# KrArunT/whisper-rust-ort

Hardware: AMD Instinct MI355X
Metric: rtfx: audio seconds transcribed per wall second (whisper-base, 30 s clips, greedy 128 new tokens) (higher is better)
Workload: dtype bf16

## Files before the change

### whisper-rust-ort_amd/csrc/wh_cross_es.hip

```cpp
#include <stdlib.h>

#include <algorithm>

#include "wh_common.h"
#include "wh_es_common.h"
#include "wh_kernels.h"

namespace {

using namespace wh_es;

constexpr int ES_D = D, ES_H = H;
constexpr int ES_ROWB = ES_D * 2;
constexpr Format ES_F = {32, 32 * ES_ROWB, 4, true, 36};

template <int AUX, int NL, int ABL = 0, bool BEAM = false>
__global__ __launch_bounds__(256 + 64 * NL, 1) void k_dec_cross_attn_es(const float* __restrict__ qe, const bf16* __restrict__ E,
                                                                         bf16* __restrict__ out, int S, int e_rows, int mpad, int B, unsigned long long* dbg,
                                                                         int rows_per_clip) {
    constexpr int TK = ES_F.tk, TILEB = ES_F.tileb, SCP = ES_F.scp;
    static_assert(NL == 1 || NL == 2, "one or two loader waves");
    extern __shared__ __attribute__((aligned(16))) char smem[];
    float* sc = carve<ES_F>(smem).sc;
    float* Qs = carve<ES_F>(smem).Qs;
// ... 187 lines not shown
#pragma unroll
        for (int u = 0; u < 8; u++) {
            const float v = u < 4 ? a[u & 3] : b[u & 3];
            const bf16 hi = (bf16)v;
            xh[ks][u] = hi;
            xl[ks][u] = (bf16)(v - (float)hi);
        }
    }
    const bf16* wp = wkT + ((long)h * d + n0 + fl) * WH_HEAD_DIM + 8 * fg;
    bf16x8 wf[8][2];
#pragma unroll
    for (int nt = 0; nt < 8; nt++)
#pragma unroll
        for (int ks = 0; ks < 2; ks++) wf[nt][ks] = *reinterpret_cast<const bf16x8*>(wp + (long)nt * 16 * WH_HEAD_DIM + 32 * ks);
#pragma unroll
    for (int nt = 0; nt < 8; nt++) {
        f32x4 acc = {0, 0, 0, 0};
#pragma unroll
        for (int ks = 0; ks < 2; ks++) {
            acc = __builtin_amdgcn_mfma_f32_16x16x32_bf16(wf[nt][ks], xl[ks], acc, 0, 0, 0);
            acc = __builtin_amdgcn_mfma_f32_16x16x32_bf16(wf[nt][ks], xh[ks], acc, 0, 0, 0);
        }
        if (m < M) *reinterpret_cast<f32x4*>(qe + ((long)m * n_heads + h) * d + n0 + 16 * nt + 4 * fg) = acc;
    }
}


constexpr int E2_ROWB = 2 * ES_D * 2;
constexpr Format E2_F = {16, 16 * E2_ROWB, 4, true, 20};

template <int AUX, int NL>
__global__ __launch_bounds__(256 + 64 * NL, 1) void k_dec_cross_attn_es2(const float* __restrict__ qe, const _Float16* __restrict__ E,
                                                                          h2* __restrict__ out, int S, int e_rows, int mpad, int B) {
    constexpr int TK = E2_F.tk, TILEB = E2_F.tileb, SCP = E2_F.scp;
    static_assert(NL == 1 || NL == 2, "one or two loader waves");
    extern __shared__ __attribute__((aligned(16))) char smem[];
    float* sc = carve<E2_F>(smem).sc;
    float* Qs = carve<E2_F>(smem).Qs;
    const int tid = threadIdx.x, lane = tid & 63;
    const int wave = __builtin_amdgcn_readfirstlane(tid >> 6);
    Walk<E2_F> w(S, B);

    if (wave >= 4) {
        constexpr int PPT = 2 * TK / NL;
        const int lw = wave - 4;
        int voff[PPT];
// ... 167 lines not shown
        for (int ks = 0; ks < 2; ks++) wf[nt][ks] = load_frag<h2>(wp + (long)nt * 16 * WH_HEAD_DIM + 32 * ks);
#pragma unroll
    for (int nt = 0; nt < 8; nt++) {
        f32x4 acc = {0, 0, 0, 0};
#pragma unroll
        for (int ks = 0; ks < 2; ks++) mma16(acc, wf[nt][ks], xs[ks]);
        if (m < M) *reinterpret_cast<f32x4*>(qe + ((long)m * n_heads + h) * d + n0 + 16 * nt + 4 * fg) = acc;
    }
}

}

#ifdef WH_ES_BENCH
unsigned long long* wh_es_bench_dbg = nullptr;
#endif

bool wh_cross_es_geometry(int d, int n_heads, int S) { return d == ES_D && n_heads == ES_H && S >= 4 * ES_F.tk; }

void wh_launch_layernorm_es2(hipStream_t s, const float* x, const float* w, const float* b, void* y, long rows, int in_blk, int out_blk) {
    hipLaunchKernelGGL(k_layernorm_es2, dim3((unsigned)((rows + 3) / 4)), dim3(256), 0, s, x, w, b, (_Float16*)y, rows, in_blk, out_blk);
}

void wh_launch_dec_cross_attn_es(hipStream_t s, int prec, const float* qe, const void* E, void* out, int S, int e_rows, int B, int mpad, bool stream_nt, int n_cus,
                                 int rows_per_clip) {
    static const int nt_env = env_int("WH_CROSS_NT", -1);
    static const int nl = env_int("WH_ES_LOADERS", 1);
    static const int persist = env_int("WH_ES_PERSIST", 1);
    if (prec == WH_PREC_FP8) { wh_launch_dec_cross_attn_es8(s, qe, E, out, S, e_rows, B, mpad, stream_nt, n_cus); return; }
    if (prec == WH_PREC_F16X3 && wh_es3_enabled()) { wh_launch_dec_cross_attn_es3(s, qe, E, out, S, e_rows, B, mpad, stream_nt, n_cus); return; }
    if (nt_env >= 0) stream_nt = nt_env != 0;
    const int grid = persist ? persistent_grid(B, n_cus) : B;
    if (prec == WH_PREC_F16X3) {
        launch(s, grid, nl == 2, stream_nt, E2_F.lds(), [](auto AUX, auto NL) { return k_dec_cross_attn_es2<decltype(AUX)::value, decltype(NL)::value>; },
               qe, (const _Float16*)E, (h2*)out, S, e_rows, mpad, B);
        return;
    }
    unsigned long long* es_dbg = nullptr;
#ifdef WH_ES_BENCH
    es_dbg = wh_es_bench_dbg;
    if (const char* e = getenv("WH_ES_ABL")) {
        const bool stamps = atoi(e) == 2;
        launch(s, grid, false, true, ES_F.lds(), [stamps](auto, auto) { return stamps ? k_dec_cross_attn_es<2, 1, 2> : k_dec_cross_attn_es<2, 1, 1>; },
               qe, (const bf16*)E, (bf16*)out, S, e_rows, mpad, B, es_dbg, 1);
        return;
    }
#endif
    if (rows_per_clip != 1) {
        launch(s, grid, nl == 2, stream_nt, ES_F.lds(), [](auto AUX, auto NL) { return k_dec_cross_attn_es<decltype(AUX)::value, decltype(NL)::value, 0, true>; },
               qe, (const bf16*)E, (bf16*)out, S, e_rows, mpad, B, es_dbg, rows_per_clip);
        return;
    }
    launch(s, grid, nl == 2, stream_nt, ES_F.lds(), [](auto AUX, auto NL) { return k_dec_cross_attn_es<decltype(AUX)::value, decltype(NL)::value>; },
           qe, (const bf16*)E, (bf16*)out, S, e_rows, mpad, B, es_dbg, 1);
}

void wh_launch_dec_qexpand(hipStream_t s, int prec, const float* q, const void* wkT, float* qe, int M, int d, int n_heads) {
    if (prec == WH_PREC_F16X3) {
        hipLaunchKernelGGL(k_dec_qexpand_x3, dim3((M + 63) / 64, n_heads, d / 128), dim3(256), 0, s, q, (const h2*)wkT, qe, M, d, n_heads);
        return;
    }
    hipLaunchKernelGGL(k_dec_qexpand, dim3((M + 63) / 64, n_heads, d / 128), dim3(256), 0, s, q, (const bf16*)wkT, qe, M, d, n_heads);
}
```

### whisper-rust-ort_amd/csrc/wh_cross_es3.hip

```cpp
#include <stdlib.h>

#include <algorithm>

#include "wh_common.h"
#include "wh_es_common.h"
#include "wh_kernels.h"

namespace {

using namespace wh_es;

constexpr int E3_D = D, E3_H = H;
constexpr int E3_ROWB = E3_D * 3;
constexpr Format E3_F = {32, 32 * E3_ROWB, 3, false, 36};
constexpr int E3_LO = E3_F.tk * E3_D * 2;
constexpr float E3_S8 = 1.0f / 4096.0f;

__device__ __forceinline__ unsigned e3_h2(float a, float b) {
    typedef __attribute__((ext_vector_type(2))) _Float16 f16x2;
    const f16x2 v = {(_Float16)a, (_Float16)b};
    unsigned u;
    __builtin_memcpy(&u, &v, 4);
    return u;
}
// ... 188 lines not shown
    }
}

__global__ __launch_bounds__(256) void k_layernorm_es3(const float* __restrict__ x, const float* __restrict__ w, const float* __restrict__ b,
                                                       unsigned char* __restrict__ y, long rows, int in_blk, int out_blk) {
    layernorm_row(x, w, b, rows, in_blk, out_blk, [&](long orow, int c, const f32x8& o) {
        f16x8 hi;
        float rm[8];
#pragma unroll
        for (int e = 0; e < 8; e++) { hi[e] = (_Float16)o[e]; rm[e] = fminf(fmaxf((o[e] - (float)hi[e]) * 4096.0f, -448.0f), 448.0f); }
        unsigned char* yr = y + orow * E3_ROWB;
        *reinterpret_cast<f16x8*>(yr + c * 2) = hi;
        *reinterpret_cast<wh_u32x2*>(yr + 2 * E3_D + c) = wh_u32x2{pack4(rm[0], rm[1], rm[2], rm[3]), pack4(rm[4], rm[5], rm[6], rm[7])};
    });
}

}

bool wh_es3_enabled() {
    static const bool on = [] { const char* e = getenv("WH_ES3"); return !(e && atoi(e) == 0); }();
    return on;
}

void wh_launch_dec_cross_attn_es3(hipStream_t s, const float* qe, const void* E, void* out, int S, int e_rows, int B, int mpad, bool stream_nt, int n_cus) {
    static const int nl = env_int("WH_ES3_LOADERS", 2);
    launch(s, persistent_grid(B, n_cus), nl != 1, stream_nt, E3_F.lds(), [](auto AUX, auto NL) { return k_dec_cross_attn_es3<decltype(AUX)::value, decltype(NL)::value>; },
           qe, (const unsigned char*)E, (h2*)out, S, e_rows, mpad, B);
}

void wh_launch_layernorm_es3(hipStream_t s, const float* x, const float* w, const float* b, void* y, long rows, int in_blk, int out_blk) {
    hipLaunchKernelGGL(k_layernorm_es3, dim3((unsigned)((rows + 3) / 4)), dim3(256), 0, s, x, w, b, (unsigned char*)y, rows, in_blk, out_blk);
}
```

### whisper-rust-ort_amd/csrc/wh_cross_es8.hip

```cpp
#include <stdlib.h>

#include <algorithm>

#include "wh_common.h"
#include "wh_es_common.h"
#include "wh_kernels.h"

namespace {

using namespace wh_es;

constexpr int E8_D = D;
constexpr int E8_ROWB = E8_D;
constexpr Format E8_F = {32, 32 * E8_ROWB, 5, true, 36};

template <int AUX, int NL>
__global__ __launch_bounds__(256 + 64 * NL, 1) void k_dec_cross_attn_es8(const float* __restrict__ qe, const unsigned char* __restrict__ E, bf16* __restrict__ out,
                                                                int S, int e_rows, int mpad, int B) {
    constexpr int TK = E8_F.tk, TILEB = E8_F.tileb, SCP = E8_F.scp;
    extern __shared__ __attribute__((aligned(16))) char smem[];
    float* sc = carve<E8_F>(smem).sc;
    float* Qs = carve<E8_F>(smem).Qs;
    const int tid = threadIdx.x, lane = tid & 63;
    const int wave = __builtin_amdgcn_readfirstlane(tid >> 6);
// ... 141 lines not shown
    const f32x4 a = *reinterpret_cast<const f32x4*>(xr), b = *reinterpret_cast<const f32x4*>(xr + 4);
    float s = 0.0f;
#pragma unroll
    for (int u = 0; u < 4; u++) s += a[u] + b[u];
    const float mean = wave_sum(s) * (1.0f / E8_D);
    float q = 0.0f;
#pragma unroll
    for (int u = 0; u < 4; u++) { q += (a[u] - mean) * (a[u] - mean); q += (b[u] - mean) * (b[u] - mean); }
    const float rstd = rsqrtf(wave_sum(q) * (1.0f / E8_D) + 1e-5f);
    const f32x4 g0 = *reinterpret_cast<const f32x4*>(gamma + lane * 8), g1 = *reinterpret_cast<const f32x4*>(gamma + lane * 8 + 4);
    const f32x4 c0 = *reinterpret_cast<const f32x4*>(beta + lane * 8), c1 = *reinterpret_cast<const f32x4*>(beta + lane * 8 + 4);
    float v[8];
#pragma unroll
    for (int u = 0; u < 4; u++) { v[u] = (a[u] - mean) * rstd * g0[u] + c0[u]; v[4 + u] = (b[u] - mean) * rstd * g1[u] + c1[u]; }
#pragma unroll
    for (int u = 0; u < 8; u++) v[u] = fminf(fmaxf(v[u], -448.0f), 448.0f);
    const wh_u32x2 o = {pack4(v[0], v[1], v[2], v[3]), pack4(v[4], v[5], v[6], v[7])};
    const long clip = r / S, key = r % S;
    *reinterpret_cast<wh_u32x2*>(out + (clip * e_rows + key) * E8_D + lane * 8) = o;
}

}

void wh_launch_dec_cross_attn_es8(hipStream_t s, const float* qe, const void* E, void* out, int S, int e_rows, int B, int mpad, bool stream_nt, int n_cus) {
    static const int nl = env_int("WH_ES8_LOADERS", 1);
    launch(s, persistent_grid(B, n_cus), nl != 1, stream_nt, E8_F.lds(), [](auto AUX, auto NL) { return k_dec_cross_attn_es8<decltype(AUX)::value, decltype(NL)::value>; },
           qe, (const unsigned char*)E, (bf16*)out, S, e_rows, mpad, B);
}

void wh_launch_layernorm_es8(hipStream_t s, const float* x, const float* gamma, const float* beta, void* out, long rows, int S, int e_rows) {
    hipLaunchKernelGGL(k_layernorm_es8, dim3((unsigned)((rows + 3) / 4)), dim3(256), 0, s, x, gamma, beta, (unsigned char*)out, rows, S, e_rows);
}
```

### whisper-rust-ort_amd/csrc/wh_ctx.cpp

```cpp
#include "wh_host_shared.h"

using namespace wh;

namespace wh {

int fail(wh_ctx* c, int code, const char* fmt, ...) {
    char buf[1024];
    va_list ap;
    va_start(ap, fmt);
    vsnprintf(buf, sizeof buf, fmt, ap);
    va_end(ap);
    if (c) c->err = buf;
    wh_set_error("%s", buf);
    return code;
}

void prof_reset(wh_ctx* c) {
    for (int g = 0; g < WH_KG_COUNT; g++) { c->prof_used[g] = 0; c->prof_ms[g] = 0; c->prof_launches[g] = 0; }
}
void prof_collect(wh_ctx* c) {
    if (!c->prof) return;
    for (int g = 0; g < WH_KG_COUNT; g++) {
        double ms = 0;
        for (size_t i = 0; i < c->prof_used[g]; i++) {
// ... 119 lines not shown
        (opts->dec_cu_mask_words && mask_bits(opts->dec_cu_mask, opts->dec_cu_mask_words) == 0)) {
        wh_set_error("wh_ctx_create_ex: a CU mask with no bit set would leave its stream without compute units");
        return WH_ERR_ARG;
    }
    auto xcds_covered = [](const uint32_t* w, size_t n) { unsigned seen = 0; for (size_t i = 0; i < n * 32; i++) if (w[i >> 5] >> (i & 31) & 1) seen |= 1u << (i & 7); return seen == 0xFFu; };
    if ((opts->enc_cu_mask_words && !xcds_covered(opts->enc_cu_mask, opts->enc_cu_mask_words)) ||
        (opts->dec_cu_mask_words && !xcds_covered(opts->dec_cu_mask, opts->dec_cu_mask_words))) {
        wh_set_error("wh_ctx_create_ex: a CU mask must select at least one compute unit of every XCD (bit i = compute unit i / 8 of XCD i %% 8)");
        return WH_ERR_ARG;
    }
    WH_HIP_CHECK(hipSetDevice(m->device));
    int n_cus = 0;
    WH_HIP_CHECK(hipDeviceGetAttribute(&n_cus, hipDeviceAttributeMultiprocessorCount, m->device));
    const bool enc_masked = opts->enc_cu_mask_words && (int)mask_bits(opts->enc_cu_mask, opts->enc_cu_mask_words) < n_cus;
    const bool dec_masked = opts->dec_cu_mask_words && (int)mask_bits(opts->dec_cu_mask, opts->dec_cu_mask_words) < n_cus;
    auto* c = new wh_ctx();
    c->m = m;
    c->max_batch = max_batch;
    c->dec_cus = dec_masked ? (int)mask_bits(opts->dec_cu_mask, opts->dec_cu_mask_words) : n_cus;
    if (dec_masked) c->dec_mask.assign(opts->dec_cu_mask, opts->dec_cu_mask + opts->dec_cu_mask_words);
    if (const char* e = getenv("WH_DEC_SPLIT")) c->split_mode = atoi(e) != 0;
    if (const char* e = getenv("WH_DEC_SPLIT_ROWS")) c->split_rows = std::max(0, atoi(e));
    if (const char* e = getenv("WH_DEC_SPLIT_CUS")) c->split_cus = std::max(1, atoi(e));
    if (const char* e = getenv("WH_DEC_FREE")) c->free_mode = atoi(e) != 0;
    if (const char* e = getenv("WH_DEC_FREE_EB")) c->free_eb = atoi(e) != 0;
    c->no_graph = getenv("WH_NO_GRAPH") != nullptr;
    c->sync_every_pos = getenv("WH_SYNC_EVERY_POS") != nullptr;
    c->al.timing = getenv("WH_ALIGN_TIMING") != nullptr;
    c->bm.timing = getenv("WH_BEAM_TIMING") != nullptr;
    c->sm.timing = getenv("WH_SAMPLE_TIMING") != nullptr;
    c->sc.timing = getenv("WH_SCORE_TIMING") != nullptr;
    const wh_dims& D = m->dims;
    const size_t B = max_batch, d = D.d_model, S = D.n_audio_ctx, F = D.ffn, C = D.n_mels, esz = m->esz;
    const size_t Ld = D.dec_layers, H = D.n_heads, TC = D.n_text_ctx;
    c->ldv = (int)align_up(S, 64);
    c->tok_ld = D.n_text_ctx + 1;
    c->mpad = (int)align_up(B, B > 16 ? 64 : 16);
    c->cross_splits = (int)std::min<size_t>(32, std::max<size_t>(1, 256 / B));
    if (m->prec == WH_PREC_BF16 && d > 512 && d % 256 == 0)
        c->cross_splits = (int)std::min<size_t>(32, std::max<size_t>(1, 512 / (B * (d / 256))));
    const size_t n_tiles = (D.vocab + 15) / 16;
    Carver cv;
    const size_t o_pcm = cv.take(B * WH_CLIP_SAMPLES * 4), o_raw = cv.take(B * C * RAW_LD * 4);
    const size_t o_melstage = cv.take(C * WH_N_FRAMES * 4);
    const size_t o_melT = cv.take((B * TOK_ROWS * C + 256) * esz), o_h1 = cv.take((B * H1_ROWS * d + 256) * esz);
    const size_t o_x = cv.take(B * S * d * 4), o_xn = cv.take(B * S * d * esz), o_qk = cv.take(B * S * 2 * d * esz);
// ... 200 lines not shown

int wh_ctx_cross_mode(const wh_ctx* c) { return c ? (c->cross_es ? 1 : 0) : -1; }

extern "C" int wh_debug_set_es_pad(wh_ctx* c, int pad_rows) {
    if (!c || !c->cross_es || pad_rows < 0 || c->m->dims.n_audio_ctx + pad_rows > c->es_rows_cap) return WH_ERR_ARG;
    c->es_rows = c->m->dims.n_audio_ctx + pad_rows;
    c->have_enc = false;
    return WH_OK;
}

extern "C" int wh_debug_set_step_split(wh_ctx* c, int rows) {
    if (!c || rows < 0) return WH_ERR_ARG;
    c->dbg_split = rows;
    return WH_OK;
}
extern "C" int wh_debug_get_step_split(const wh_ctx* c) { return c ? c->last_split : -1; }
extern "C" int wh_debug_set_step_free(wh_ctx* c, int on) {
    if (!c) return WH_ERR_ARG;
    c->dbg_free = on != 0;
    return WH_OK;
}
extern "C" int wh_debug_get_step_free(const wh_ctx* c) { return c ? c->last_free : -1; }

const char* wh_last_error(const wh_ctx* c) { return c ? c->err.c_str() : wh_global_error().c_str(); }

int wh_get_timings(const wh_ctx* c, wh_timing* out) {
    if (!c || !out) return WH_ERR_ARG;
    *out = c->timing;
    return WH_OK;
}

int wh_profile_enable(wh_ctx* c, int group_mask) {
    if (!c) return WH_ERR_ARG;
    c->prof = (group_mask & 0xFFFF) != 0;
    c->prof_mask = group_mask & 0xFFFF;
    c->prof_stride = (group_mask >> 16) & 0xFFFF;
    return WH_OK;
}
int wh_profile_get(const wh_ctx* c, double* ms, int64_t* launches) {
    if (!c || !ms || !launches) return WH_ERR_ARG;
    for (int g = 0; g < WH_KG_COUNT; g++) { ms[g] = c->prof_ms[g]; launches[g] = c->prof_launches[g]; }
    return WH_OK;
}

}
```

### whisper-rust-ort_amd/csrc/wh_es_common.h

```cpp
#pragma once
#include <stdlib.h>

#include <algorithm>
#include <type_traits>

#include "wh_common.h"
#include "wh_kernels.h"

namespace wh_es {

typedef const __attribute__((address_space(1))) void* gptr_t;
typedef __attribute__((address_space(3))) void* lptr_t;

constexpr int D = 512, H = 8;
constexpr float LOG2E = 1.44269504088896341f;
constexpr float REM = 16.0f, REM_INV = 1.0f / 16.0f;

template <int N> __device__ __forceinline__ void wait_vm() { asm volatile("s_waitcnt vmcnt(%0)" ::"n"(N) : "memory"); }
template <int AUX>
__device__ __forceinline__ void glds16(const void* src, char* lds_wave_base) {
    __builtin_amdgcn_global_load_lds((gptr_t)src, (lptr_t)lds_wave_base, 16, 0, AUX);
}
__device__ __forceinline__ int swz8(int r) { return (r & 15) ^ (((r >> 4) & 1) << 3); }
__device__ __forceinline__ float ror8(float v) {
// ... 215 lines not shown
}

template <typename Store>
__device__ __forceinline__ void layernorm_row(const float* __restrict__ x, const float* __restrict__ w, const float* __restrict__ b, long rows, int in_blk, int out_blk, Store store) {
    const long row = (long)blockIdx.x * 4 + (threadIdx.x >> 6);
    if (row >= rows) return;
    const int lane = threadIdx.x & 63, c = lane * 8;
    const float* xr = x + row * D;
    const f32x4 v0 = __builtin_nontemporal_load(reinterpret_cast<const f32x4*>(xr + c)), v1 = __builtin_nontemporal_load(reinterpret_cast<const f32x4*>(xr + c + 4));
    const float mean = dpp_wave_sum((v0[0] + v0[1] + v0[2] + v0[3]) + (v1[0] + v1[1] + v1[2] + v1[3])) / (float)D;
    float q = 0.0f;
#pragma unroll
    for (int e = 0; e < 4; e++) { const float t0 = v0[e] - mean, t1 = v1[e] - mean; q += t0 * t0; q += t1 * t1; }
    const float rstd = rsqrtf(dpp_wave_sum(q) / (float)D + 1e-5f);
    const f32x4 w0 = *reinterpret_cast<const f32x4*>(w + c), w1 = *reinterpret_cast<const f32x4*>(w + c + 4);
    const f32x4 b0 = *reinterpret_cast<const f32x4*>(b + c), b1 = *reinterpret_cast<const f32x4*>(b + c + 4);
    f32x8 o;
#pragma unroll
    for (int e = 0; e < 4; e++) { o[e] = (v0[e] - mean) * rstd * w0[e] + b0[e]; o[4 + e] = (v1[e] - mean) * rstd * w1[e] + b1[e]; }
    store(in_blk > 0 ? (row / in_blk) * out_blk + row % in_blk : row, c, o);
}

inline int env_int(const char* name, int dflt) { const char* e = getenv(name); return e ? atoi(e) : dflt; }
inline int persistent_grid(int B, int n_cus) { return std::min(B, n_cus <= 0 ? 256 : n_cus); }
template <typename Pick, typename... Args>
void launch(hipStream_t s, int grid, bool two_loaders, bool stream_nt, int lds, Pick pick, Args... args) {
    wh_with_flags([&](auto NT, auto TWO) {
        constexpr int AUX = decltype(NT)::value ? 2 : 0, NL = decltype(TWO)::value ? 2 : 1;
        void (*kfn)(Args...) = pick(std::integral_constant<int, AUX>{}, std::integral_constant<int, NL>{});
        wh_ensure_dyn_lds((const void*)kfn, lds);
        hipLaunchKernelGGL(kfn, dim3(grid), dim3(256 + 64 * NL), lds, s, args...);
    }, stream_nt, two_loaders);
}

}
```

### whisper-rust-ort_amd/csrc/wh_internal.h

```cpp
#pragma once
#include <hip/hip_runtime.h>

#include <array>
#include <map>
#include <string>
#include <tuple>
#include <vector>

#include "../../include/whisper_hip.h"
#include "wh_kernels.h"

struct EncLayerDev {
    void *qk_w, *v_w, *o_w, *fc1_w, *fc2_w;
    float *qk_b, *v_b, *o_b, *fc1_b, *fc2_b;
    float *ln1_w, *ln1_b, *ln2_w, *ln2_b;
    float *qk_sc = nullptr, *v_sc = nullptr, *o_sc = nullptr, *fc1_sc = nullptr, *fc2_sc = nullptr;
    void *qk_w8 = nullptr, *v_w8 = nullptr, *fc1_w8 = nullptr, *fc2_w8 = nullptr;
    void *qk_wf = nullptr, *v_wf = nullptr, *fc1_wf = nullptr;
    float *qk_s = nullptr, *qk_c = nullptr, *v_s = nullptr, *v_c = nullptr, *fc1_s = nullptr, *fc1_c = nullptr;
};
struct DecLayerDev {
    void *qkv_w, *o_w, *cq_w, *co_w, *fc1_w, *fc2_w;
    float *qkv_b, *o_b, *cq_b, *co_b, *fc1_b, *fc2_b;
    float *ln1_w, *ln1_b, *ln2_w, *ln2_b, *ln3_w, *ln3_b;
// ... 41 lines not shown
    operator T*() const { return (T*)p; }
};

template <size_t N>
void wh_drain_events(std::vector<std::array<hipEvent_t, N>>& events, double* ms) {
    for (auto& te : events) {
        for (size_t i = 0; ms && i + 1 < N; i++) { float t = 0; hipEventElapsedTime(&t, te[i], te[i + 1]); ms[i] += t; }
        for (auto& e : te) hipEventDestroy(e);
    }
    events.clear();
}

struct wh_ctx {
    wh_model* m = nullptr;
    int max_batch = 1;
    int dec_cus = 256;
    hipStream_t stream = nullptr;
    hipStream_t s_enc = nullptr;
    hipStream_t cur = nullptr;
    hipStream_t s_split = nullptr;
    std::vector<hipEvent_t> split_ev;
    std::vector<uint32_t> dec_mask;
    int split_mode = -1, split_rows = 0, split_cus = 160, dbg_split = 0, last_split = 0;
    std::vector<hipEvent_t> free_ev;
    int free_mode = -1, dbg_free = 0, last_free = 0;
    bool free_eb = true;
    hipEvent_t ev_enc_done = nullptr, ev_kv_done = nullptr;
    bool kv_done_armed = false;
    hipEvent_t enc_ev[2][3] = {{nullptr}};
    int enc_set = 0;
    const float* pre_pcm = nullptr;
    int pre_n = 0;
    bool pre_valid = false;
    std::string err;
    wh_timing timing{};
    bool have_enc = false;
    int enc_batch = 0;
    bool prof = false;
    int prof_mask = 0;
    int prof_stride = 0;
    bool capturing = false;
    bool no_graph = false;
    bool sync_every_pos = false;
    int prof_group = -1;
    std::vector<std::pair<hipEvent_t, hipEvent_t>> prof_events[WH_KG_COUNT];
    size_t prof_used[WH_KG_COUNT] = {0};
// ... 282 lines not shown
```

### whisper-rust-ort_amd/csrc/wh_kernels.h

```cpp
#pragma once
#include <hip/hip_runtime.h>
#include <stddef.h>
#include <vector>

#include "../../include/whisper_hip.h"

constexpr int WH_SMALL_CTX_CLIPS = 8;

struct GemmArgs {
    const void* A = nullptr;
    long lda = 0, a_bs = 0, a_zs = 0;
    const void* W = nullptr;
    long ldw = 0, w_zs = 0;
    void* C = nullptr;
    long ldc = 0, c_bs = 0, c_zs = 0;
    const float* bias = nullptr;
    int bias_mode = 0;
    const float* wscale = nullptr;
    const float* R = nullptr;
    long ldr = 0, r_bs = 0, r_zs = 0;
    int act = 0;
    int M = 0, N = 0, K = 0;
    int m_per = 1 << 30;
    int n_per = 1 << 30;
// ... 199 lines not shown
    const void* X = nullptr;
    int x_mpad = 64;
    const void* W = nullptr;
    const float* bias = nullptr;
    const float* ln_s = nullptr;
    const float* ln_part = nullptr;
    int ln_tiles = 0;
    const int* ids = nullptr;
    int n_lang = 0;
    int M = 0, K = 0;
    float* out = nullptr;
};
void wh_launch_lang_head(hipStream_t s, int prec, const LangHeadArgs& a);
void wh_launch_lang_finish(hipStream_t s, const float* logits, const int* ids, int n_lang, int src_row, float* probs, int* chosen, int* feed,
                           int* out_tokens, int tok_ld, int tok_pos, int B, int* pos_p);
void wh_launch_dec_self_attn(hipStream_t s, int prec, const void* qkv, void* kc, void* vc, void* out, const int* pos_p,
                             int d, int n_heads, int tc, int B, int mpad, const int* off = nullptr);
void wh_launch_dec_cross_attn(hipStream_t s, int prec, const void* q, const void* ck, const void* cv, float* part,
                              float* ml, int S, int d, int n_heads, int splits, int B, void* out, int mpad, bool stream_nt,
                              int rows_per_clip = 1);

bool wh_cross_es_geometry(int d, int n_heads, int S);
void wh_launch_dec_qexpand(hipStream_t s, int prec, const float* q, const void* wkT, float* qe, int M, int d, int n_heads);
void wh_launch_dec_cross_attn_es(hipStream_t s, int prec, const float* qe, const void* E, void* out, int S, int e_rows, int B, int mpad, bool stream_nt, int n_cus,
                                 int rows_per_clip = 1);
void wh_launch_layernorm_es2(hipStream_t s, const float* x, const float* w, const float* b, void* y, long rows, int in_blk, int out_blk);
bool wh_es3_enabled();
void wh_launch_dec_cross_attn_es3(hipStream_t s, const float* qe, const void* E, void* out, int S, int e_rows, int B, int mpad, bool stream_nt, int n_cus);
void wh_launch_layernorm_es3(hipStream_t s, const float* x, const float* w, const float* b, void* y, long rows, int in_blk, int out_blk);
void wh_launch_dec_cross_attn_es8(hipStream_t s, const float* qe, const void* E, void* out, int S, int e_rows, int B, int mpad, bool stream_nt, int n_cus);
void wh_launch_layernorm_es8(hipStream_t s, const float* x, const float* gamma, const float* beta, void* out, long rows, int S, int e_rows);

size_t wh_cross_lds_reserve(long total_wgs, size_t own_bytes);

void wh_launch_kv_quant(hipStream_t s, const void* kv_bf16, unsigned* amax, void* kv8, long planes_x_clips, int S, int d,
                        int n_heads);
void wh_launch_dec_cross_attn8(hipStream_t s, const void* q, const void* ck, const void* cv, const float* amax_k,
                               const float* amax_v, float* part, float* ml, int S, int d, int n_heads, int splits, int B, void* out,
                               int mpad, bool stream_nt);

struct AlignLayerHeads {
    int n = 0;
    unsigned char slot[WH_MAX_ALIGN_HEADS] = {0}, head[WH_MAX_ALIGN_HEADS] = {0};
};
void wh_launch_align_copy(hipStream_t s, bool src_bf16, const void* src, long row_pitch, long head_pitch, int dk, const AlignLayerHeads& hs, const int* pos_p,
                          int first_emit, int cap, int nb, float* dst);
constexpr int WH_ALIGN_KV_F32 = 0, WH_ALIGN_KV_BF16 = 1, WH_ALIGN_ES_BF16 = 2;
struct AlignArgs {
    const float* q = nullptr;
    const void* k_base[WH_MAX_ALIGN_HEADS] = {nullptr};
    long k_clip_pitch = 0, k_row_pitch = 0;
    int dk = 0;
    const int* n_out = nullptr;
// ... 72 lines not shown
```

### whisper-rust-ort_amd/csrc/wh_step.h

```cpp
#pragma once
#include "wh_host_shared.h"

namespace wh {

void pack_mask(const int64_t* a, size_t na, const int64_t* b, size_t nb, int vocab, std::vector<unsigned>& out);
int project_cross_kv(wh_ctx* c, int nb, const std::function<int()>& after_kv);

struct StepBase {
    wh_ctx* c;
    const wh_ctx::StepKey& k;
    wh_model* m = c->m;
    const wh_dims& D = m->dims;
    hipStream_t s = c->stream;
    const int prec = m->prec, nb = k.nb, mpad = c->mpad, ln_tiles_d = D.d_model / 16;
    const long d = D.d_model, S = D.n_audio_ctx;
    const bool f8 = prec == WH_PREC_FP8, rules = k.ts_begin >= 0;
    const int rpc, ncl, clip0;
    const bool kv_nt = (c->cross_es ? 1.0 : (double)D.dec_layers * 2.0) * ncl * S * d * (f8 ? 1 : (double)m->esz) > 128.0 * 1024 * 1024;
    int row0 = 0, nr = nb, es_cus = c->dec_cus;
    int *pos = c->pos, *ticket = c->step_ticket;
    template <typename T> T* rm(T* p, long ld) const { return p + (long)row0 * ld; }
    void* rm(void* p, long ld, size_t esz) const { return (char*)p + (long)row0 * ld * (long)esz; }
    void* slab(void* p) const { return (char*)p + (long)row0 * 32 * (long)m->esz; }
    hipEvent_t q_rec = nullptr;
// ... 40 lines not shown
    template <typename SelfAttn>
    void layer_with(int l, bool advance, SelfAttn&& self_attn) const {
        layer_head(l, self_attn);
        layer_tail(l, advance);
    }
    template <typename SelfAttn>
    void layer_head(int l, SelfAttn&& self_attn) const {
        const DecLayerDev& L = m->dec[l];
        {
            Prof pr(c, WH_KG_DEC_GEMM);
            gemm(false, ln_consumer(L.qkv_w, L.qkv_b, L.qkv_sc, L.qkv_s, 3 * d, rm(c->dqkv, 3 * d, prec == WH_PREC_F16X3 ? 4 : m->esz), (l == 0) ? 1 : ln_tiles_d));
        }
        {
            Prof pr(c, WH_KG_DEC_OTHER);
            self_attn();
        }
        {
            Prof pr(c, WH_KG_DEC_GEMM);
            gemm(true, residual_producer(L.o_w, L.o_b, L.o_sc, slab(c->datt), d, L.ln2_w));
        }
        if (c->cross_es) {
            {
                Prof pr(c, WH_KG_DEC_GEMM);
                gemm(true, ln_consumer(L.cq_w, L.cq_b, L.cq_sc, L.cq_s, d, rm(c->dq32, d), ln_tiles_d));
                wh_launch_dec_qexpand(s, prec, rm(c->dq32, d), L.cqx_w, rm(c->dqe, D.n_heads * d), nr, (int)d, D.n_heads);
            }
        } else {
            Prof pr(c, WH_KG_DEC_GEMM);
            gemm(false, ln_consumer(L.cq_w, L.cq_b, L.cq_sc, L.cq_s, d, rm(c->dq, d, prec == WH_PREC_F16X3 ? 4 : m->esz), ln_tiles_d));
        }
        after_query(l);
    }
    void layer_tail(int l, bool advance) const {
        const DecLayerDev& L = m->dec[l];
        const long kv_stride = (long)ncl * S * d;
        const long kv_clip0 = (long)(clip0 + row0) * S * d;
        if (c->cross_es) {
            if (k.al_q && c->al.layer[l].n) {
                Prof pr(c, WH_KG_DEC_OTHER);
                wh_launch_align_copy(s, false, c->dqe, (long)D.n_heads * d, d, (int)d, c->al.layer[l], c->pos, k.n_prompt - 1, k.al_cap, nb, k.al_q);
            }
            {
                Prof pr(c, WH_KG_DEC_CROSS_ATTN);
                wh_launch_dec_cross_attn_es(s, prec, rm(c->dqe, D.n_heads * d), (const char*)c->es_E + (long)(clip0 + row0) * c->es_rows * d * m->esz, slab(c->dctx), (int)S,
                                            c->es_rows, nr, mpad, kv_nt, es_cus, rpc);
            }
            {
                Prof pr(c, WH_KG_DEC_GEMM);
                SkinnyArgs a;
                a.X = slab(c->dctx); a.x_mpad = mpad; a.W = L.cv_w; a.bias = L.cv_b; a.C = slab(c->datt); a.c_mpad = mpad;
                a.M = nr; a.m_sel = nb; a.N = WH_HEAD_DIM; a.K = (int)d;
                a.zn = D.n_heads; a.x_zs = (long)(d / 32) * mpad * 32; a.w_zs = (long)WH_HEAD_DIM * d; a.c_zs = (long)(WH_HEAD_DIM / 32) * mpad * 32;
                a.bias_zs = WH_HEAD_DIM;
                if (f8) wh_launch_dec_gemm(s, WH_PREC_BF16, false, a);
                else gemm(false, a);
            }
        } else {
            if (k.al_q && c->al.layer[l].n) {
                Prof pr(c, WH_KG_DEC_OTHER);
                wh_launch_align_copy(s, m->esz == 2, c->dq, d, WH_HEAD_DIM, WH_HEAD_DIM, c->al.layer[l], c->pos, k.n_prompt - 1, k.al_cap, nb, k.al_q);
            }
            Prof pr(c, WH_KG_DEC_CROSS_ATTN);
            if (f8)
                wh_launch_dec_cross_attn8(s, c->dq, (char*)c->cross_kv8 + (2 * l) * kv_stride, (char*)c->cross_kv8 + (2 * l + 1) * kv_stride,
                                          c->kv_amax + (long)(2 * l) * nb * D.n_heads, c->kv_amax + (long)(2 * l + 1) * nb * D.n_heads,
                                          c->cpart, c->cml, (int)S, (int)d, D.n_heads, c->cross_splits, nb, c->datt, mpad, kv_nt);
            else
                wh_launch_dec_cross_attn(s, prec, rm(c->dq, d, prec == WH_PREC_F16X3 ? 4 : m->esz), (char*)c->cross_kv + ((2 * l) * kv_stride + kv_clip0) * m->esz,
// ... 28 lines not shown
```

Measured before the change: 80620.

## Fuse LN-folded cross-attention query GEMM with per-head query expansion

Adds a kernel that computes the LayerNorm-folded cross-attention query projection for one head's 64 columns and immediately expands it through the key weights, replacing a skinny GEMM launch plus a separate qexpand launch. The intermediate query no longer round-trips through global memory and one launch per decoder layer is removed. It is on by default for bf16 when tiled decode is off. It also adds an opt-in whole-rounds persistent-grid sizing for the cross-attention kernel, along with a debug check and a trace summary script.

```diff
diff --git a/profiles/range_trace_summary.py b/profiles/range_trace_summary.py
--- /dev/null
+++ b/profiles/range_trace_summary.py
@@ -0,0 +1,63 @@
+import csv
+import sys
+from collections import Counter
+
+
+def main():
+    path = sys.argv[1]
+    n_pos = int(sys.argv[2]) if len(sys.argv) > 2 else 127
+    rows = []
+    with open(path, newline="") as f:
+        for r in csv.DictReader(f):
+            wg = int(r.get("Workgroup_Size_X") or r.get("Workgroup_Size") or 1)
+            gr = int(r.get("Grid_Size_X") or r.get("Grid_Size") or 0)
+            rows.append((int(r["Start_Timestamp"]), int(r["End_Timestamp"]), r["Kernel_Name"], gr // max(1, wg)))
+    rows.sort()
+    es = [r for r in rows if "k_dec_cross_attn_es" in r[2]]
+    if not es:
+        print("no k_dec_cross_attn_es dispatch in the trace")
+        return
+    widest = max(r[3] for r in es)
+    rng = [r for r in es if r[3] < widest]
+    print(f"{len(rows)} dispatches, {len(es)} of k_dec_cross_attn_es; grids (workgroups: launches): {dict(sorted(Counter(r[3] for r in es).items()))}")
+    loops, cur = [], []
+    for r in rng:
+        if cur and r[0] - cur[-1][1] > 20_000_000:
+            loops.append(cur)
+            cur = []
+        cur.append(r)
+    if cur:
+        loops.append(cur)
+    for li, lp in enumerate(loops):
+        t0, t1 = lp[0][0], max(r[1] for r in lp)
+        inside = [r for r in rows if r[0] >= t0 and r[1] <= t1]
+        covered, end = 0, t0
+        for s, e, _, _ in lp:
+            if e > end:
+                covered += e - max(s, end)
+                end = e
+        alone, beside = [], []
+        for i, (s, e, _, _) in enumerate(lp):
+            ov = 0
+            for j in range(max(0, i - 4), min(len(lp), i + 5)):
+                if j != i:
+                    ov += max(0, min(e, lp[j][1]) - max(s, lp[j][0]))
+            (beside if 2 * ov > e - s else alone).append((e - s) / 1e3)
+        names = Counter(r[2].split("(")[0][:60] for r in inside)
+        mean = lambda v: sum(v) / len(v) if v else float("nan")
+        print(f"loop {li}: {len(lp)} range launches, window {(t1 - t0) / 1e6:.1f} ms, {n_pos} positions")
+        print(f"  kernels per generated position                  {len(inside) / n_pos:.1f}")
+        print(f"  first-to-last kernel span per position, us      {(t1 - t0) / 1e3 / n_pos:,.1f}")
+        print(f"  kernel time summed per position, us             {sum(r[1] - r[0] for r in inside) / 1e3 / n_pos:,.1f}")
+        print(f"  no k_dec_cross_attn_es running, us per position {(t1 - t0 - covered) / 1e3 / n_pos:,.1f}")
+        print(f"  range launches alone: {len(alone)}, mean {mean(alone):.1f} us; beside another for more than half their time: {len(beside)}, mean {mean(beside):.1f} us")
+        for k in ("k_dec_cq_expand", "k_dec_qexpand", "k_dec_gemm_wide", "k_dec_gemm<"):
+            sel = [r for r in inside if k in r[2]]
+            if sel:
+                print(f"  {k:<18} {len(sel):6d} launches, mean {mean([(r[1] - r[0]) / 1e3 for r in sel]):.2f} us")
+        if li == 0:
+            print("  dispatches by kernel:", ", ".join(f"{n.split('<')[0].split('::')[-1]} {c}" for n, c in names.most_common(14)))
+
+
+if __name__ == "__main__":
+    main()
diff --git a/whisper-rust-ort_amd/csrc/wh_cross_es.hip b/whisper-rust-ort_amd/csrc/wh_cross_es.hip
--- a/whisper-rust-ort_amd/csrc/wh_cross_es.hip
+++ b/whisper-rust-ort_amd/csrc/wh_cross_es.hip
@@ -233,6 +233,122 @@
             acc = __builtin_amdgcn_mfma_f32_16x16x32_bf16(wf[nt][ks], xh[ks], acc, 0, 0, 0);
         }
         if (m < M) *reinterpret_cast<f32x4*>(qe + ((long)m * n_heads + h) * d + n0 + 16 * nt + 4 * fg) = acc;
+    }
+}
+
+template <int MT>
+struct CqxLds {
+    static constexpr int TILES = 4 * MT, ROWS = 16 * MT, QP = 68;
+    static constexpr size_t RED = (size_t)4 * TILES * 64 * 16, LNQ = (size_t)4 * ROWS * 2 * 4, QB = (size_t)ROWS * QP * 4, BYTES = RED + LNQ + QB;
+};
+
+template <int MT>
+__global__ __launch_bounds__(512) void k_dec_cq_expand(SkinnyArgs a, const bf16* __restrict__ wkT, float* __restrict__ qe, int n_heads) {
+    static_assert(MT == 2 || MT == 4, "a wave expands whole groups of eight column tiles");
+    extern __shared__ __attribute__((aligned(16))) char cqx_smem[];
+    typedef CqxLds<MT> Lds;
+    constexpr int TILES = Lds::TILES, ROWS = Lds::ROWS, QP = Lds::QP;
+    f32x4* red = reinterpret_cast<f32x4*>(cqx_smem);
+    float* lnq = reinterpret_cast<float*>(cqx_smem + Lds::RED);
+    float* Q = reinterpret_cast<float*>(cqx_smem + Lds::RED + Lds::LNQ);
+    const int tid = threadIdx.x, lane = tid & 63, wave = tid >> 6, fl = lane & 15, fg = lane >> 4;
+    const int h = blockIdx.y, m0 = blockIdx.x * ROWS, d = a.N;
+    {
+        const int kq = wave & 3, ch = wave >> 2;
+        const bf16* wp = (const bf16*)a.W + (long)(h * WH_HEAD_DIM + 32 * ch + fl) * a.K + 128 * kq + 8 * fg;
+        const bf16* xp = (const bf16*)a.X + (long)(4 * kq) * a.x_mpad * 32 + 8 * fg;
+        bf16x8 wq[4][2], xq[4][MT];
+#pragma unroll
+        for (int i = 0; i < 4; i++) {
+#pragma unroll
+            for (int c = 0; c < 2; c++) wq[i][c] = load_frag<bf16>(wp + (long)c * 16 * a.K + 32 * i);
+#pragma unroll
+            for (int t = 0; t < MT; t++) xq[i][t] = load_frag<bf16>(xp + ((long)i * a.x_mpad + min(m0 + 16 * t + fl, a.M - 1)) * 32);
+        }
+        if (tid < 4 * ROWS) {
+            const int r = tid % ROWS, q = tid / ROWS;
+            float s1, s2;
+            ln_partial_sum(a.ln_part, a.ln_tiles, a.x_mpad, min(m0 + r, a.M - 1), q, 4, s1, s2);
+            ln_part_store<ROWS>(lnq, r, q, s1, s2);
+        }
+        f32x4 acc[2][MT];
+#pragma unroll
+        for (int c = 0; c < 2; c++)
+#pragma unroll
+            for (int t = 0; t < MT; t++) acc[c][t] = f32x4{0, 0, 0, 0};
+#pragma unroll
+        for (int i = 0; i < 4; i++)
+#pragma unroll
+            for (int c = 0; c < 2; c++)
+#pragma unroll
+                for (int t = 0; t < MT; t++) mma16(acc[c][t], wq[i][c], xq[i][t]);
+#pragma unroll
+        for (int c = 0; c < 2; c++)
+#pragma unroll
+            for (int t = 0; t < MT; t++) red[(kq * TILES + (2 * ch + c) * MT + t) * 64 + lane] = acc[c][t];
+    }
+    __syncthreads();
+#pragma unroll
+    for (int j = 0; j < TILES / 8; j++) {
+        const int t = wave + 8 * j, ct = t / MT, mt = t % MT;
+        const int en = h * WH_HEAD_DIM + 16 * ct + 4 * fg, em = m0 + 16 * mt + fl;
+        f32x4 s = red[t * 64 + lane];
+#pragma unroll
+        for (int w = 1; w < 4; w++) {
+            const f32x4 o = red[(w * TILES + t) * 64 + lane];
+            s[0] += o[0]; s[1] += o[1]; s[2] += o[2]; s[3] += o[3];
+        }
+        float ln_mean, ln_rstd;
+        ln_row_stats<ROWS>(lnq, 16 * mt + fl, a.K, ln_mean, ln_rstd);
+        f32x4 pre_bias = {0, 0, 0, 0}, pre_ws = {1, 1, 1, 1};
+        if (a.bias) pre_bias = *reinterpret_cast<const f32x4*>(a.bias + en);
+        if (a.wscale) pre_ws = *reinterpret_cast<const f32x4*>(a.wscale + en);
+        const f32x4 pre_sv = *reinterpret_cast<const f32x4*>(a.ln_s + en);
+        f32x4 v;
+#pragma unroll
+        for (int e = 0; e < 4; e++) {
+            v[e] = wh_ln_fold(wh_scale(s[e], pre_ws[e]), ln_mean, ln_rstd, pre_sv[e], pre_bias[e]);
+            v[e] += 0.0f;
+        }
+        *reinterpret_cast<f32x4*>(Q + (16 * mt + fl) * QP + 16 * ct + 4 * fg) = v;
+        if (a.shift_io && h == 0 && ct == 0 && fg == 0 && em < a.M) a.shift_io[em] += ln_mean;
+    }
+    __syncthreads();
+    {
+        const int rt = wave % MT, nb0 = (wave / MT) * (4 * MT * 16);
+        const int m = m0 + 16 * rt + fl;
+        bf16x8 xh[2], xl[2];
+#pragma unroll
+        for (int ks = 0; ks < 2; ks++) {
+            const float* qp = Q + (16 * rt + fl) * QP + 32 * ks + 8 * fg;
+            const f32x4 qa = *reinterpret_cast<const f32x4*>(qp), qb = *reinterpret_cast<const f32x4*>(qp + 4);
+#pragma unroll
+            for (int u = 0; u < 8; u++) {
+                const float v = u < 4 ? qa[u & 3] : qb[u & 3];
+                const bf16 hi = (bf16)v;
+                xh[ks][u] = hi;
+                xl[ks][u] = (bf16)(v - (float)hi);
+            }
+        }
+#pragma unroll
+        for (int n0 = nb0; n0 < nb0 + 4 * MT * 16; n0 += 128) {
+            const bf16* wp = wkT + ((long)h * d + n0 + fl) * WH_HEAD_DIM + 8 * fg;
+            bf16x8 wf[8][2];
+#pragma unroll
+            for (int nt = 0; nt < 8; nt++)
+#pragma unroll
+                for (int ks = 0; ks < 2; ks++) wf[nt][ks] = *reinterpret_cast<const bf16x8*>(wp + (long)nt * 16 * WH_HEAD_DIM + 32 * ks);
+#pragma unroll
+            for (int nt = 0; nt < 8; nt++) {
+                f32x4 acc = {0, 0, 0, 0};
+#pragma unroll
+                for (int ks = 0; ks < 2; ks++) {
+                    acc = __builtin_amdgcn_mfma_f32_16x16x32_bf16(wf[nt][ks], xl[ks], acc, 0, 0, 0);
+                    acc = __builtin_amdgcn_mfma_f32_16x16x32_bf16(wf[nt][ks], xh[ks], acc, 0, 0, 0);
+                }
+                if (m < a.M) *reinterpret_cast<f32x4*>(qe + ((long)m * n_heads + h) * d + n0 + 16 * nt + 4 * fg) = acc;
+            }
+        }
     }
 }
 
@@ -446,14 +562,14 @@
 }
 
 void wh_launch_dec_cross_attn_es(hipStream_t s, int prec, const float* qe, const void* E, void* out, int S, int e_rows, int B, int mpad, bool stream_nt, int n_cus,
-                                 int rows_per_clip) {
+                                 int rows_per_clip, bool whole_rounds) {
     static const int nt_env = env_int("WH_CROSS_NT", -1);
     static const int nl = env_int("WH_ES_LOADERS", 1);
     static const int persist = env_int("WH_ES_PERSIST", 1);
-    if (prec == WH_PREC_FP8) { wh_launch_dec_cross_attn_es8(s, qe, E, out, S, e_rows, B, mpad, stream_nt, n_cus); return; }
-    if (prec == WH_PREC_F16X3 && wh_es3_enabled()) { wh_launch_dec_cross_attn_es3(s, qe, E, out, S, e_rows, B, mpad, stream_nt, n_cus); return; }
+    if (prec == WH_PREC_FP8) { wh_launch_dec_cross_attn_es8(s, qe, E, out, S, e_rows, B, mpad, stream_nt, n_cus, whole_rounds); return; }
+    if (prec == WH_PREC_F16X3 && wh_es3_enabled()) { wh_launch_dec_cross_attn_es3(s, qe, E, out, S, e_rows, B, mpad, stream_nt, n_cus, whole_rounds); return; }
     if (nt_env >= 0) stream_nt = nt_env != 0;
-    const int grid = persist ? persistent_grid(B, n_cus) : B;
+    const int grid = persist ? persistent_grid(B, n_cus, whole_rounds) : B;
     if (prec == WH_PREC_F16X3) {
         launch(s, grid, nl == 2, stream_nt, E2_F.lds(), [](auto AUX, auto NL) { return k_dec_cross_attn_es2<decltype(AUX)::value, decltype(NL)::value>; },
                qe, (const _Float16*)E, (h2*)out, S, e_rows, mpad, B);
@@ -485,3 +601,20 @@
     }
     hipLaunchKernelGGL(k_dec_qexpand, dim3((M + 63) / 64, n_heads, d / 128), dim3(256), 0, s, q, (const bf16*)wkT, qe, M, d, n_heads);
 }
+
+void wh_launch_dec_cq_expand(hipStream_t s, const SkinnyArgs& a, const void* wkT, float* qe, int n_heads, int row_tiles) {
+    if (a.K != ES_D || a.N != ES_D || n_heads != ES_H || !a.ln_part || !a.ln_s || a.R || a.act || a.zn != 1 || a.xpart || a.ticket) {
+        fprintf(stderr, "wh_launch_dec_cq_expand: not the LN2-folded cross-attention query of the %d x %d geometry\n", ES_D, ES_H);
+        abort();
+    }
+    static const int mt_env = env_int("WH_CQX_MT", 0);
+    const int mt = row_tiles == 2 || row_tiles == 4 ? row_tiles : mt_env == 2 || mt_env == 4 ? mt_env : (a.M >= 2048 ? 4 : 2);
+    wh_with_pow2<2, 4>(mt, [&](auto MTC) {
+        constexpr int MT = decltype(MTC)::value;
+        auto kfn = k_dec_cq_expand<MT>;
+        wh_ensure_dyn_lds((const void*)kfn, (int)CqxLds<MT>::BYTES);
+        hipLaunchKernelGGL(kfn, dim3((a.M + 16 * MT - 1) / (16 * MT), n_heads), dim3(512), CqxLds<MT>::BYTES, s, a, (const bf16*)wkT, qe, n_heads);
+    });
+}
+
+extern "C" int wh_debug_es_grid(int B, int cap, int whole_rounds) { return persistent_grid(B, cap, whole_rounds != 0); }
diff --git a/whisper-rust-ort_amd/csrc/wh_cross_es3.hip b/whisper-rust-ort_amd/csrc/wh_cross_es3.hip
--- a/whisper-rust-ort_amd/csrc/wh_cross_es3.hip
+++ b/whisper-rust-ort_amd/csrc/wh_cross_es3.hip
@@ -234,9 +234,9 @@
     return on;
 }
 
-void wh_launch_dec_cross_attn_es3(hipStream_t s, const float* qe, const void* E, void* out, int S, int e_rows, int B, int mpad, bool stream_nt, int n_cus) {
+void wh_launch_dec_cross_attn_es3(hipStream_t s, const float* qe, const void* E, void* out, int S, int e_rows, int B, int mpad, bool stream_nt, int n_cus, bool whole_rounds) {
     static const int nl = env_int("WH_ES3_LOADERS", 2);
-    launch(s, persistent_grid(B, n_cus), nl != 1, stream_nt, E3_F.lds(), [](auto AUX, auto NL) { return k_dec_cross_attn_es3<decltype(AUX)::value, decltype(NL)::value>; },
+    launch(s, persistent_grid(B, n_cus, whole_rounds), nl != 1, stream_nt, E3_F.lds(), [](auto AUX, auto NL) { return k_dec_cross_attn_es3<decltype(AUX)::value, decltype(NL)::value>; },
            qe, (const unsigned char*)E, (h2*)out, S, e_rows, mpad, B);
 }
 
diff --git a/whisper-rust-ort_amd/csrc/wh_cross_es8.hip b/whisper-rust-ort_amd/csrc/wh_cross_es8.hip
--- a/whisper-rust-ort_amd/csrc/wh_cross_es8.hip
+++ b/whisper-rust-ort_amd/csrc/wh_cross_es8.hip
@@ -187,9 +187,9 @@
 
 }
 
-void wh_launch_dec_cross_attn_es8(hipStream_t s, const float* qe, const void* E, void* out, int S, int e_rows, int B, int mpad, bool stream_nt, int n_cus) {
+void wh_launch_dec_cross_attn_es8(hipStream_t s, const float* qe, const void* E, void* out, int S, int e_rows, int B, int mpad, bool stream_nt, int n_cus, bool whole_rounds) {
     static const int nl = env_int("WH_ES8_LOADERS", 1);
-    launch(s, persistent_grid(B, n_cus), nl != 1, stream_nt, E8_F.lds(), [](auto AUX, auto NL) { return k_dec_cross_attn_es8<decltype(AUX)::value, decltype(NL)::value>; },
+    launch(s, persistent_grid(B, n_cus, whole_rounds), nl != 1, stream_nt, E8_F.lds(), [](auto AUX, auto NL) { return k_dec_cross_attn_es8<decltype(AUX)::value, decltype(NL)::value>; },
            qe, (const unsigned char*)E, (bf16*)out, S, e_rows, mpad, B);
 }
 
diff --git a/whisper-rust-ort_amd/csrc/wh_ctx.cpp b/whisper-rust-ort_amd/csrc/wh_ctx.cpp
--- a/whisper-rust-ort_amd/csrc/wh_ctx.cpp
+++ b/whisper-rust-ort_amd/csrc/wh_ctx.cpp
@@ -165,6 +165,8 @@
     if (const char* e = getenv("WH_DEC_SPLIT")) c->split_mode = atoi(e) != 0;
     if (const char* e = getenv("WH_DEC_SPLIT_ROWS")) c->split_rows = std::max(0, atoi(e));
     if (const char* e = getenv("WH_DEC_SPLIT_CUS")) c->split_cus = std::max(1, atoi(e));
+    if (const char* e = getenv("WH_ES_ROUNDS")) c->es_rounds = atoi(e) != 0;
+    if (const char* e = getenv("WH_DEC_CQX")) c->cqx = atoi(e) != 0;
     if (const char* e = getenv("WH_DEC_FREE")) c->free_mode = atoi(e) != 0;
     if (const char* e = getenv("WH_DEC_FREE_EB")) c->free_eb = atoi(e) != 0;
     c->no_graph = getenv("WH_NO_GRAPH") != nullptr;
@@ -411,6 +413,63 @@
 }
 extern "C" int wh_debug_get_step_free(const wh_ctx* c) { return c ? c->last_free : -1; }
 
+extern "C" int wh_debug_cq_expand_check(int M, int row0, int pitch, int m_sel, int fused, unsigned long long* hashes, long* n_bad) {
+    if (M < 1 || row0 < 0 || pitch % 16 || row0 + M > pitch || !hashes || !n_bad) return -1;
+    constexpr int d = 512, H = 8, LT = d / 16;
+    unsigned st = 12345u;
+    auto rnd = [&]() { st = st * 1664525u + 1013904223u; return (float)(st >> 8) * (1.0f / 8388608.0f) - 1.0f; };
+    auto to_bf16 = [](float f) { unsigned u; __builtin_memcpy(&u, &f, 4); u += 0x7FFFu + ((u >> 16) & 1u); return (unsigned short)(u >> 16); };
+    auto from_bf16 = [](unsigned short b) { const unsigned u = (unsigned)b << 16; float f; __builtin_memcpy(&f, &u, 4); return f; };
+    std::vector<unsigned short> X((size_t)(d / 32) * pitch * 32), W((size_t)d * d), WK((size_t)H * d * 64);
+    std::vector<float> part((size_t)LT * pitch * 2, 0.0f), bias(d), lns(d), shift(pitch);
+    for (int m = 0; m < pitch; m++)
+        for (int k = 0; k < d; k++) {
+            const unsigned short b = to_bf16(25.0f + rnd());
+            X[((size_t)(k >> 5) * pitch + m) * 32 + (k & 31)] = b;
+            const float v = from_bf16(b);
+            part[((size_t)(k >> 4) * pitch + m) * 2] += v;
+            part[((size_t)(k >> 4) * pitch + m) * 2 + 1] += v * v;
+        }
+    for (auto& w : W) w = to_bf16(0.05f * rnd());
+    for (auto& w : WK) w = to_bf16(0.1f * rnd());
+    for (int n = 0; n < d; n++) { bias[n] = rnd(); lns[n] = 0.02f * rnd(); }
+    const size_t qe_n = (size_t)pitch * H * d;
+    std::vector<unsigned char> qe_h(qe_n * 4, 0xA5), sh_h((size_t)pitch * 4, 0xA5);
+    for (int m = row0; m < row0 + M; m++) { const float v = 3.0f + m; __builtin_memcpy(&sh_h[(size_t)m * 4], &v, 4); }
+    void *dX = nullptr, *dW = nullptr, *dWK = nullptr, *dpart = nullptr, *dbias = nullptr, *dlns = nullptr, *dsh = nullptr, *dq = nullptr, *dqe = nullptr;
+    auto up = [](void** p, const void* h, size_t bytes) { return hipMalloc(p, bytes) == hipSuccess && hipMemcpy(*p, h, bytes, hipMemcpyHostToDevice) == hipSuccess; };
+    bool ok = up(&dX, X.data(), X.size() * 2) && up(&dW, W.data(), W.size() * 2) && up(&dWK, WK.data(), WK.size() * 2) && up(&dpart, part.data(), part.size() * 4) &&
+              up(&dbias, bias.data(), d * 4) && up(&dlns, lns.data(), d * 4) && up(&dsh, sh_h.data(), sh_h.size()) && up(&dqe, qe_h.data(), qe_h.size()) &&
+              hipMalloc(&dq, (size_t)pitch * d * 4) == hipSuccess && hipMemset(dq, 0xA5, (size_t)pitch * d * 4) == hipSuccess;
+    if (ok) {
+        SkinnyArgs a;
+        a.X = (const unsigned short*)dX + (size_t)row0 * 32; a.x_mpad = pitch; a.W = dW; a.bias = (const float*)dbias;
+        a.C = (float*)dq + (size_t)row0 * d; a.ldc = d; a.M = M; a.m_sel = m_sel; a.N = d; a.K = d;
+        a.ln_part = (const float*)dpart + (size_t)row0 * 2; a.ln_tiles = LT; a.ln_s = (const float*)dlns; a.shift_io = (float*)dsh + row0;
+        float* qe = (float*)dqe + (size_t)row0 * H * d;
+        if (fused) wh_launch_dec_cq_expand(0, a, dWK, qe, H, fused);
+        else {
+            wh_launch_dec_gemm(0, WH_PREC_BF16, true, a);
+            wh_launch_dec_qexpand(0, WH_PREC_BF16, (const float*)a.C, dWK, qe, M, d, H);
+        }
+        ok = hipDeviceSynchronize() == hipSuccess && hipMemcpy(qe_h.data(), dqe, qe_h.size(), hipMemcpyDeviceToHost) == hipSuccess &&
+             hipMemcpy(sh_h.data(), dsh, sh_h.size(), hipMemcpyDeviceToHost) == hipSuccess;
+    }
+    for (void* p : {dX, dW, dWK, dpart, dbias, dlns, dsh, dq, dqe}) if (p) hipFree(p);
+    if (!ok) return -2;
+    auto fnv = [](const std::vector<unsigned char>& v) { unsigned long long h = 1469598103934665603ull; for (unsigned char c : v) { h ^= c; h *= 1099511628211ull; } return h; };
+    hashes[0] = fnv(qe_h);
+    hashes[1] = fnv(sh_h);
+    long bad = 0;
+    for (int m = 0; m < pitch; m++) {
+        if (m >= row0 && m < row0 + M) continue;
+        for (size_t i = (size_t)m * H * d * 4; i < (size_t)(m + 1) * H * d * 4; i++) bad += qe_h[i] != 0xA5;
+        for (size_t i = (size_t)m * 4; i < (size_t)(m + 1) * 4; i++) bad += sh_h[i] != 0xA5;
+    }
+    *n_bad = bad;
+    return 0;
+}
+
 const char* wh_last_error(const wh_ctx* c) { return c ? c->err.c_str() : wh_global_error().c_str(); }
 
 int wh_get_timings(const wh_ctx* c, wh_timing* out) {
diff --git a/whisper-rust-ort_amd/csrc/wh_es_common.h b/whisper-rust-ort_amd/csrc/wh_es_common.h
--- a/whisper-rust-ort_amd/csrc/wh_es_common.h
+++ b/whisper-rust-ort_amd/csrc/wh_es_common.h
@@ -261,7 +261,12 @@
 }
 
 inline int env_int(const char* name, int dflt) { const char* e = getenv(name); return e ? atoi(e) : dflt; }
-inline int persistent_grid(int B, int n_cus) { return std::min(B, n_cus <= 0 ? 256 : n_cus); }
+inline int persistent_grid(int B, int cap, bool whole_rounds = false) {
+    if (cap <= 0) cap = 256;
+    if (B <= cap || !whole_rounds) return std::min(B, cap);
+    const int r = (B + cap - 1) / cap;
+    return (B + r - 1) / r;
+}
 template <typename Pick, typename... Args>
 void launch(hipStream_t s, int grid, bool two_loaders, bool stream_nt, int lds, Pick pick, Args... args) {
     wh_with_flags([&](auto NT, auto TWO) {
diff --git a/whisper-rust-ort_amd/csrc/wh_internal.h b/whisper-rust-ort_amd/csrc/wh_internal.h
--- a/whisper-rust-ort_amd/csrc/wh_internal.h
+++ b/whisper-rust-ort_amd/csrc/wh_internal.h
@@ -87,6 +87,7 @@
     std::vector<hipEvent_t> split_ev;
     std::vector<uint32_t> dec_mask;
     int split_mode = -1, split_rows = 0, split_cus = 160, dbg_split = 0, last_split = 0;
+    bool es_rounds = false, cqx = true;
     std::vector<hipEvent_t> free_ev;
     int free_mode = -1, dbg_free = 0, last_free = 0;
     bool free_eb = true;
diff --git a/whisper-rust-ort_amd/csrc/wh_kernels.h b/whisper-rust-ort_amd/csrc/wh_kernels.h
--- a/whisper-rust-ort_amd/csrc/wh_kernels.h
+++ b/whisper-rust-ort_amd/csrc/wh_kernels.h
@@ -245,13 +245,14 @@
 
 bool wh_cross_es_geometry(int d, int n_heads, int S);
 void wh_launch_dec_qexpand(hipStream_t s, int prec, const float* q, const void* wkT, float* qe, int M, int d, int n_heads);
+void wh_launch_dec_cq_expand(hipStream_t s, const SkinnyArgs& a, const void* wkT, float* qe, int n_heads, int row_tiles = 0);
 void wh_launch_dec_cross_attn_es(hipStream_t s, int prec, const float* qe, const void* E, void* out, int S, int e_rows, int B, int mpad, bool stream_nt, int n_cus,
-                                 int rows_per_clip = 1);
+                                 int rows_per_clip = 1, bool whole_rounds = false);
 void wh_launch_layernorm_es2(hipStream_t s, const float* x, const float* w, const float* b, void* y, long rows, int in_blk, int out_blk);
 bool wh_es3_enabled();
-void wh_launch_dec_cross_attn_es3(hipStream_t s, const float* qe, const void* E, void* out, int S, int e_rows, int B, int mpad, bool stream_nt, int n_cus);
+void wh_launch_dec_cross_attn_es3(hipStream_t s, const float* qe, const void* E, void* out, int S, int e_rows, int B, int mpad, bool stream_nt, int n_cus, bool whole_rounds = false);
 void wh_launch_layernorm_es3(hipStream_t s, const float* x, const float* w, const float* b, void* y, long rows, int in_blk, int out_blk);
-void wh_launch_dec_cross_attn_es8(hipStream_t s, const float* qe, const void* E, void* out, int S, int e_rows, int B, int mpad, bool stream_nt, int n_cus);
+void wh_launch_dec_cross_attn_es8(hipStream_t s, const float* qe, const void* E, void* out, int S, int e_rows, int B, int mpad, bool stream_nt, int n_cus, bool whole_rounds = false);
 void wh_launch_layernorm_es8(hipStream_t s, const float* x, const float* gamma, const float* beta, void* out, long rows, int S, int e_rows);
 
 size_t wh_cross_lds_reserve(long total_wgs, size_t own_bytes);
diff --git a/whisper-rust-ort_amd/csrc/wh_step.h b/whisper-rust-ort_amd/csrc/wh_step.h
--- a/whisper-rust-ort_amd/csrc/wh_step.h
+++ b/whisper-rust-ort_amd/csrc/wh_step.h
@@ -86,8 +86,13 @@
         if (c->cross_es) {
             {
                 Prof pr(c, WH_KG_DEC_GEMM);
-                gemm(true, ln_consumer(L.cq_w, L.cq_b, L.cq_sc, L.cq_s, d, rm(c->dq32, d), ln_tiles_d));
-                wh_launch_dec_qexpand(s, prec, rm(c->dq32, d), L.cqx_w, rm(c->dqe, D.n_heads * d), nr, (int)d, D.n_heads);
+                const SkinnyArgs a = ln_consumer(L.cq_w, L.cq_b, L.cq_sc, L.cq_s, d, rm(c->dq32, d), ln_tiles_d);
+                if (c->cqx && prec == WH_PREC_BF16 && !c->dec_tile) {
+                    wh_launch_dec_cq_expand(s, a, L.cqx_w, rm(c->dqe, D.n_heads * d), D.n_heads);
+                } else {
+                    gemm(true, a);
+                    wh_launch_dec_qexpand(s, prec, rm(c->dq32, d), L.cqx_w, rm(c->dqe, D.n_heads * d), nr, (int)d, D.n_heads);
+                }
             }
         } else {
             Prof pr(c, WH_KG_DEC_GEMM);
@@ -107,7 +112,7 @@
             {
                 Prof pr(c, WH_KG_DEC_CROSS_ATTN);
                 wh_launch_dec_cross_attn_es(s, prec, rm(c->dqe, D.n_heads * d), (const char*)c->es_E + (long)(clip0 + row0) * c->es_rows * d * m->esz, slab(c->dctx), (int)S,
-                                            c->es_rows, nr, mpad, kv_nt, es_cus, rpc);
+                                            c->es_rows, nr, mpad, kv_nt, es_cus, rpc, c->es_rounds);
             }
             {
                 Prof pr(c, WH_KG_DEC_GEMM);
```

Result: no change. 81540 (median of 6 runs) (+1.1%).
